# jimmyyhwu/spatial-intention-maps

Measured on AMD Instinct MI355X. Metric: Q-map transitions/sec, 96x96: `value` = full train() step (M2: policy fwd + bwd, double-DQN next-state forwards, clip, SGD); `value_fwd_bwd_only` = policy fwd+bwd alone (M1, the literal reading of "fwd+bwd"), higher is better.
Workload: dtype f32

## Files before the change

### include/simq.h

```cpp
#ifndef SIMQ_H
#define SIMQ_H

#include <stdint.h>

#ifdef __cplusplus
extern "C" {
#endif

#define SIMQ_VERSION 500
#define SIMQ_STATE_WIDTH 96

#define SIMQ_MODE_EVAL 0
#define SIMQ_MODE_TRAIN 1
#define SIMQ_MODE_TRAIN_NOGRAD 2

#define SIMQ_KIND_CONV_W 0
#define SIMQ_KIND_CONV_B 1
#define SIMQ_KIND_BN_W 2
#define SIMQ_KIND_BN_B 3

#define SIMQ_PREC_FP32 0
#define SIMQ_PREC_BF16X3 1
#define SIMQ_PREC_BF16 2

// ... 144 lines not shown
int simq_comm_broadcast(simq_comm* comm, void* d_buf, int64_t bytes, int root, void* producer_stream);
int simq_comm_wait(simq_comm* comm, void* consumer_stream);
int simq_comm_progress(simq_comm* comm, int64_t out[4]);
int simq_comm_time_waits(simq_comm* comm, int on);
int simq_comm_last_wait_ms(simq_comm* comm, float* ms);
int simq_comm_destroy(simq_comm* comm);

int simq_bce_with_logits(const float* d_logits, const float* d_target, int64_t n, float* d_dlogits, double* d_loss_sum, void* stream);
int simq_split_last_channel(const float* d_x, float* d_head, float* d_last, int64_t pixels, int channels, void* stream);
int simq_sigmoid_concat(const float* d_state, const float* d_logit, float* d_out, float* d_prob, int64_t pixels, int channels, void* stream);

int simq_nchw_to_nhwc(const float* d_in, float* d_out, int batch, int channels, int hw, void* stream);
int simq_nhwc_to_nchw(const float* d_in, float* d_out, int batch, int channels, int hw, void* stream);

typedef struct simq_launch_opts {
    int struct_bytes;
    int force_bm, force_bn;
    int tail_split;
    int plane_xcd;
    int wgrad_xcd_group;
    int wgrad_ksplit;
    int gemm_split;
} simq_launch_opts;
void simq_launch_opts_default(simq_launch_opts* opts);
int simq_conv2d_fwd(const float* d_x, const float* d_w_ohwi, const float* d_bias, float* d_y,
                    int batch, int hin, int win, int cin, int cout, int r, int s, int stride, int pad,
                    double* d_stats , void* stream, const simq_launch_opts* opts);
int simq_conv2d_fwd_winograd(const float* d_x, const float* d_w_ohwi, const float* d_bias, float* d_y,
                             int batch, int hin, int win, int cin, int cout,
                             double* d_stats , float* d_scratch, void* stream, const simq_launch_opts* opts);
int simq_conv2d_fwd_winograd4(const float* d_x, const float* d_w_ohwi, const float* d_bias, float* d_y,
                              int batch, int hin, int win, int cin, int cout,
                              double* d_stats , float* d_scratch, void* stream, const simq_launch_opts* opts);
int simq_bn_relu_apply(const void* d_y, const double* d_stats, const float* d_gamma, const float* d_beta, const void* d_res, int relu,
                       void* d_out, int64_t rows, int channels, int storage, float* d_saved, float* d_running, void* stream);
int simq_bn_relu_backward(const void* d_g, const void* d_mask, int mask_kind, const void* d_y, const float* d_saved, const float* d_gamma,
                          const double* d_red, void* d_dy, void* d_dz_out, float* d_dgamma, float* d_dbeta, int64_t rows, int channels,
                          int storage, void* stream);
int simq_conv2d_fwd_bnrelu_in(const float* d_y_pre, const float* d_in_scale, const float* d_in_shift, const float* d_w_ohwi,
                              const float* d_bias, float* d_y, int batch, int hin, int win, int cin, int cout, int r, int s, int stride,
                              int pad, int form, float* d_scratch, void* stream, const simq_launch_opts* opts);
int simq_conv2d_wgrad_bnrelu_in(const float* d_y_pre, const float* d_in_scale, const float* d_in_shift, const float* d_dy, float* d_dw,
                                int batch, int hin, int win, int cin, int cout, int r, int s, int stride, int pad, int form,
                                float* d_scratch, void* stream, const simq_launch_opts* opts);
int simq_conv2d_fwd_stem_f32(const float* d_x, const float* d_w_ohwi, float* d_y, int batch, int hin, int win, int cin, double* d_stats,
                             void* stream);
int simq_conv2d_fwd_stem_bf16(const float* d_x, const float* d_w_ohwi, uint16_t* d_y, int batch, int hin, int win, int cin,
                              double* d_stats, void* d_scratch, void* stream);
int simq_conv2d_wgrad_stem_bf16(const float* d_x, const uint16_t* d_dy, float* d_dw, int batch, int hin, int win, int cin,
                                float* d_scratch, void* stream);
int simq_conv2d_wgrad_winograd(const float* d_x, const float* d_dy, float* d_dw_ohwi,
                               int batch, int hin, int win, int cin, int cout, float* d_scratch, void* stream, const simq_launch_opts* opts);
int simq_gemm_f32_batched(const float* d_x, const float* d_w, float* d_y, int m, int n, int k, int batch, void* stream,
                          const simq_launch_opts* opts);
int simq_conv2d_dgrad(const float* d_dy, const float* d_w_ohwi, float* d_wt_scratch, float* d_dx,
                      int batch, int hin, int win, int cin, int cout, int r, int s, int pad, void* stream, const simq_launch_opts* opts);
int simq_conv2d_wgrad(const float* d_x, const float* d_dy, float* d_dw_ohwi ,
                      int batch, int hin, int win, int cin, int cout, int r, int s, int stride, int pad,
                      void* stream, const simq_launch_opts* opts);
int simq_conv2d_fwd_bf16(const float* d_x, const float* d_w_ohwi, const float* d_bias, float* d_y, int batch, int hin, int win,
                         int cin, int cout, int r, int s, int stride, int pad, int nplanes, void* d_scratch, double* d_stats,
                         void* stream, const simq_launch_opts* opts);
int simq_conv2d_wgrad_bf16(const float* d_x, const float* d_dy, float* d_dw_ohwi, int batch, int hin, int win, int cin, int cout,
                           int r, int s, int stride, int pad, int nplanes, void* d_scratch, void* stream, const simq_launch_opts* opts);
int64_t simq_conv2d_wgrad_bf16_slab_bytes(void);
int simq_conv2d_wgrad_bf16_slab(const float* d_x, const float* d_dy, float* d_dw_ohwi, int batch, int hin, int win, int cin, int cout,
// ... 185 lines not shown
```

### spatial-intention-maps_amd/csrc/common.h

```cpp
#pragma once
#include <hip/hip_runtime.h>
#include <stdint.h>

struct simq_comm;

namespace simq {

typedef float floatx16 __attribute__((ext_vector_type(16)));
typedef float floatx4 __attribute__((ext_vector_type(4)));

void set_error(const char* fmt, ...);

#ifdef SIMQ_ABLATIONS
int tune_env_int(const char* name, int dflt);
#define SIMQ_TUNE_INT(name, dflt) (simq::tune_env_int(name, dflt))
#else
#define SIMQ_TUNE_INT(name, dflt) (dflt)
#endif

#define SIMQ_CHECK_HIP(expr)                                                        \
    do {                                                                            \
        hipError_t _e = (expr);                                                     \
        if (_e != hipSuccess) {                                                     \
            simq::set_error("%s:%d: %s -> %s", __FILE__, __LINE__, #expr, hipGetErrorString(_e)); \
// ... 57 lines not shown
    int C = 0;
    double* defer = nullptr;
};
struct InBn {
    const float* scale = nullptr; const float* shift = nullptr;
    BnRef bn;
    int live = 0;
    bool on() const { return live != 0 || scale != nullptr; }
};

void prof_launch_begin(int kind, double flops, double bytes, hipStream_t stream);
void prof_launch_end(hipStream_t stream);
void note_launch(const char* family);

int launch_conv_igemm(const float* x, const float* w, float* y, const ConvGeom& g, const ConvEpilogue& e,
                      hipStream_t stream, const InBn& in = InBn());
int try_gemm_batched_pp(const float* x, const float* w, float* y, int M, int N, int K, int batch, hipStream_t stream);
int launch_gemm_batched(const float* x, const float* w, float* y, int M, int N, int K, int batch, hipStream_t stream, const LaunchTune& tune = LaunchTune());
bool gemm_split3_eligible(int M, int N, int K, int batch);
int launch_gemm_batched_split3(const float* x, const float* w, float* y, int M, int N, int K, int batch, hipStream_t stream, const LaunchTune& tune);
bool winograd_eligible(const ConvGeom& g);
bool winograd_pays(int cin, int cout, long min_cc);
int64_t winograd_scratch_floats(const ConvGeom& g);
int launch_wino_weight(const float* w_ohwi, float* U, int cout, int cin, hipStream_t stream);
struct WinoWeightDesc { int64_t src_off, u_off; int cout, cin, from_wt, pad_; };
constexpr int kWinoWeightTableCap = 72;
struct WinoWeightTable { WinoWeightDesc d[kWinoWeightTableCap]; int n; };
int launch_wino_weight_all(const float* params, const float* wt, float* ubase, const WinoWeightTable& t, hipStream_t stream);
int launch_conv_winograd(const float* x, const float* U, float* y, const ConvGeom& g, const ConvEpilogue& e, float* scratch,
                         hipStream_t stream, const InBn& in = InBn());
bool winograd_f4_forward(const ConvGeom& g, int min_tiles);
int launch_conv_winograd4(const float* x, const float* U4, float* y, const ConvGeom& g, const ConvEpilogue& e, float* scratch,
                          hipStream_t stream, const InBn& in = InBn());
constexpr int64_t kWgradDetSlabFloats = 16 << 20;
constexpr int kWgradMaxSplits = 96;
inline int64_t stem_det_slab_floats(int cin) {
    const int64_t want = (int64_t)kWgradMaxSplits * 64 * 49 * cin;
    return want < kWgradDetSlabFloats ? want : kWgradDetSlabFloats;
}
int launch_conv_wgrad(const float* x, const float* dy, float* dw, const ConvGeom& g, hipStream_t stream, const InBn& in = InBn(), float* det_slab = nullptr,
                      int64_t det_slab_floats = kWgradDetSlabFloats);
int launch_wgrad_slab_sum(const float* slab, float* dw, int64_t n, int splits, hipStream_t stream);
int launch_wgrad_batched(const float* x, const float* dy, float* dw, int M, int N, int K, int batch, hipStream_t stream, const LaunchTune& tune = LaunchTune());
bool winograd_wgrad_eligible(const ConvGeom& g);
bool winograd_wgrad_pays(const ConvGeom& g, bool allow_f4);
int launch_conv_wgrad_winograd(const float* x, const float* dy, float* dw, const ConvGeom& g, float* scratch, hipStream_t stream, bool allow_f4 = true,
                               const InBn& in = InBn());
int tune_forced_tile(const LaunchTune& t, int* bm, int* bn);
int launch_conv_igemm_bf16(const uint16_t* const x[2], const uint16_t* const w[2], int nplanes, float* y, const ConvGeom& g,
                           const ConvEpilogue& e, hipStream_t stream);
int launch_conv_wgrad_bf16(const uint16_t* const x[2], const uint16_t* const dy[2], int nplanes, float* dw, const ConvGeom& g,
                           hipStream_t stream, float* slab = nullptr, float* det_slab = nullptr);
int try_conv_wgrad_bf16_pp(const uint16_t* x, const uint16_t* dy, float* dw, const ConvGeom& g, unsigned x_bytes, unsigned dy_bytes,
                           hipStream_t stream);
int try_conv_wgrad_bf16_img(const uint16_t* x, const uint16_t* dy, float* dw, const ConvGeom& g, unsigned x_bytes, unsigned dy_bytes,
                           hipStream_t stream, float* slab = nullptr);
int64_t conv_wgrad_bf16_slab_bytes();
struct WeightPrepDesc { int64_t w_off, wt_off, wp_off; int cout, taps, cin, pad_; };
struct WeightPrepTable { WeightPrepDesc d[24]; int n; };
int launch_weight_prep_all(const float* params, const WeightPrepTable& t, float* wt_f32, uint16_t* wpl, uint16_t* wtpl, int np,
                           int64_t wp_total, hipStream_t stream);
int launch_split_planes(const float* src, uint16_t* hi, uint16_t* lo, int64_t n, hipStream_t stream);
int launch_weight_planes(const float* w, uint16_t* w_hi, uint16_t* w_lo, uint16_t* wt_hi, uint16_t* wt_lo, int cout, int taps,
                         int cin, hipStream_t stream);
int launch_weight_transpose(const float* w, float* wt, int cout, int taps, int cin, hipStream_t stream);

// ... 80 lines not shown
```

### spatial-intention-maps_amd/csrc/conv_winograd.hip

```cpp
#include "common.h"
#include "bn_coeff.h"
#include "igemm_epilogue.h"

namespace simq {

namespace {

__global__ void __launch_bounds__(256) wino_weight_kernel(const float* __restrict__ w, float* __restrict__ U, int cout, int cin) {
    const int total = cout * cin;
    for (int i = blockIdx.x * 256 + threadIdx.x; i < total; i += gridDim.x * 256) {
        const int co = i / cin, ci = i - co * cin;
        const float* g = w + (size_t)co * 9 * cin + ci;
        float t[4][3];
#pragma unroll
        for (int c = 0; c < 3; ++c) {
            const float g0 = g[(0 * 3 + c) * cin], g1 = g[(1 * 3 + c) * cin], g2 = g[(2 * 3 + c) * cin];
            t[0][c] = g0;
            t[1][c] = 0.5f * (g0 + g1 + g2);
            t[2][c] = 0.5f * (g0 - g1 + g2);
            t[3][c] = g2;
        }
#pragma unroll
        for (int r = 0; r < 4; ++r) {
            const float u0 = t[r][0], u1 = 0.5f * (t[r][0] + t[r][1] + t[r][2]), u2 = 0.5f * (t[r][0] - t[r][1] + t[r][2]), u3 = t[r][2];
// ... 324 lines not shown
                    }
                    s0 += dz;
                    s1 += dz * ((y1 - mu1) * is1);
                    if (bnr2) {
                        const floatx4 y2 = *reinterpret_cast<const floatx4*>(p.bnr_y2 + o);
                        s2 += dz;
                        s3 += dz * ((y2 - mu2) * is2);
                    }
                }
            }
        }
    }
    if (!p.stats && !bnr) return;
#pragma unroll
    for (int c = 0; c < 4; ++c) {
        red[0][threadIdx.x][c] = s0[c]; red[1][threadIdx.x][c] = s1[c];
        red[2][threadIdx.x][c] = s2[c]; red[3][threadIdx.x][c] = s3[c];
    }
    __syncthreads();
    for (int lc = threadIdx.x; lc < 4 * lanes; lc += 256) {
        double a0 = 0.0, a1 = 0.0, a2 = 0.0, a3 = 0.0;
        for (int k = 0; k < tpb; ++k) {
            const int src = k * lanes + (lc >> 2);
            a0 += (double)red[0][src][lc & 3]; a1 += (double)red[1][src][lc & 3];
            a2 += (double)red[2][src][lc & 3]; a3 += (double)red[3][src][lc & 3];
        }
        const int ch = blockIdx.y * lanes * 4 + lc;
        double* dst = p.stats ? p.stats : p.bnr_red1;
        unsafeAtomicAdd(dst + ch, a0);
        unsafeAtomicAdd(dst + C + ch, a1);
        if (bnr2) {
            unsafeAtomicAdd(p.bnr_red2 + ch, a2);
            unsafeAtomicAdd(p.bnr_red2 + C + ch, a3);
        }
    }
}

__global__ void __launch_bounds__(256) wino_dy_kernel(const float* __restrict__ dy, float* __restrict__ dM, int B, int H, int W, int C, int T) {
    const int lanes = C >> 2, tpb = 256 / lanes;
    const int cl = threadIdx.x % lanes, tl = threadIdx.x / lanes;
    const int th = H >> 1, tw = W >> 1;
    const size_t gstride = (size_t)T * C;
    for (int t = blockIdx.x * tpb + tl; t < T; t += gridDim.x * tpb) {
        const int b = t / (th * tw), r = t - b * (th * tw);
        const int ty = r / tw, tx = r - ty * tw;
        const float* src = dy + ((size_t)(b * H + 2 * ty) * W + 2 * tx) * C + cl * 4;
        const floatx4 y00 = *reinterpret_cast<const floatx4*>(src), y01 = *reinterpret_cast<const floatx4*>(src + C);
        const floatx4 y10 = *reinterpret_cast<const floatx4*>(src + (size_t)W * C), y11 = *reinterpret_cast<const floatx4*>(src + (size_t)W * C + C);
        floatx4 a[4][2];
        a[0][0] = y00; a[0][1] = y01;
        a[1][0] = y00 + y10; a[1][1] = y01 + y11;
        a[2][0] = y00 - y10; a[2][1] = y01 - y11;
        a[3][0] = -y10; a[3][1] = -y11;
        float* dst = dM + (size_t)t * C + cl * 4;
#pragma unroll
        for (int i = 0; i < 4; ++i) {
            *reinterpret_cast<floatx4*>(dst + (i * 4 + 0) * gstride) = a[i][0];
            *reinterpret_cast<floatx4*>(dst + (i * 4 + 1) * gstride) = a[i][0] + a[i][1];
            *reinterpret_cast<floatx4*>(dst + (i * 4 + 2) * gstride) = a[i][0] - a[i][1];
            *reinterpret_cast<floatx4*>(dst + (i * 4 + 3) * gstride) = -a[i][1];
        }
    }
}

template <bool DY, bool XBN = false>
__global__ void __launch_bounds__(256) wino_tr_kernel(const float* __restrict__ src, float* __restrict__ out, int B, int H, int W, int C, int T,
// ... 260 lines not shown
    if (bin > 4096) bin = 4096;
    if (in.on()) hipLaunchKernelGGL(wino_input_kernel<true>, dim3(bin), dim3(256), 0, stream, x, V, g.B, g.Hin, g.Win, g.Cin, T, in);
    else hipLaunchKernelGGL(wino_input_kernel<false>, dim3(bin), dim3(256), 0, stream, x, V, g.B, g.Hin, g.Win, g.Cin, T, in);
    SIMQ_CHECK_LAUNCH();
    if (int rc = launch_gemm_batched(V, U, Mt, T, g.Cout, g.Cin, 16, stream, g.tune)) return rc;
    int bout = (T + tpb_out - 1) / tpb_out;
    bout = balanced_grid(bout, (e.stats || e.bnr_red1) ? 512 : 4096);
    const EpiArgs ea = make_epi(y, e);
    note_launch("winograd_f2");
    hipLaunchKernelGGL(wino_output_kernel, dim3(bout), dim3(256), 0, stream, Mt, ea, g.B, g.Hin, g.Win, g.Cout, T);
    SIMQ_CHECK_LAUNCH();
    return 0;
}

bool winograd_f4_forward(const ConvGeom& g, int min_tiles) {
    return winograd_eligible(g) && g.Hin % 4 == 0 && g.Win % 4 == 0 && g.B * (g.Hin / 4) * (g.Win / 4) >= min_tiles;
}


int launch_conv_winograd4(const float* x, const float* U4, float* y, const ConvGeom& g, const ConvEpilogue& e, float* scratch,
                          hipStream_t stream, const InBn& in) {
    SIMQ_REQUIRE(winograd_eligible(g) && g.Hin % 4 == 0 && g.Win % 4 == 0, "conv_winograd4: geometry not supported");
    SIMQ_REQUIRE(!e.y_bf16, "conv_winograd4: fp32 outputs only");
    const int T4 = g.B * (g.Hin / 4) * (g.Win / 4);
    float* V = scratch;
    float* Mt = scratch + (size_t)36 * T4 * g.Cin;
    const int tpb_in = 256 / (g.Cin / 4);
    int bin = (T4 + tpb_in - 1) / tpb_in;
    if (bin > 4096) bin = 4096;
    if (in.on()) hipLaunchKernelGGL(wino4f_input_kernel<true>, dim3(bin), dim3(256), 0, stream, x, V, g.B, g.Hin, g.Win, g.Cin, T4, in);
    else hipLaunchKernelGGL(wino4f_input_kernel<false>, dim3(bin), dim3(256), 0, stream, x, V, g.B, g.Hin, g.Win, g.Cin, T4, in);
    SIMQ_CHECK_LAUNCH();
    if (int rc = launch_gemm_batched(V, U4, Mt, T4, g.Cout, g.Cin, 36, stream, g.tune)) return rc;
    static const int slice_quads = SIMQ_TUNE_INT("SIMQ_W4F_OUT_SLICE_QUADS", 16);
    int lanes_out = g.Cout / 4;
    if ((e.stats || e.bnr_red1) && slice_quads > 0 && lanes_out > slice_quads && lanes_out % slice_quads == 0) lanes_out = slice_quads;
    const int tpb_o = 256 / lanes_out, slices = (g.Cout / 4) / lanes_out;
    int bout = (T4 + tpb_o - 1) / tpb_o;
    bout = balanced_grid(bout, ((e.stats || e.bnr_red1) ? 1024 : 4096) / slices);
    const EpiArgs ea = make_epi(y, e);
    note_launch("winograd_f4");
    hipLaunchKernelGGL(wino4f_output_kernel, dim3(bout, slices), dim3(256), 0, stream, Mt, ea, g.B, g.Hin, g.Win, g.Cout, T4, lanes_out);
    SIMQ_CHECK_LAUNCH();
    return 0;
}

bool winograd_wgrad_eligible(const ConvGeom& g) { return winograd_eligible(g) && g.Cin % 128 == 0 && g.Cout % 128 == 0; }

bool winograd_wgrad_f4(const ConvGeom& g) {
    return g.Hin % 4 == 0 && g.Win % 4 == 0 && (g.B * (g.Hin / 4) * (g.Win / 4)) % 16 == 0;
}

bool winograd_wgrad_pays(const ConvGeom& g, bool allow_f4) {
    return (long)g.Cin * g.Cout >= ((allow_f4 && winograd_wgrad_f4(g)) ? 128L * 256 : 256L * 256);
}

int launch_conv_wgrad_winograd(const float* x, const float* dy, float* dw, const ConvGeom& g, float* scratch, hipStream_t stream, bool allow_f4,
                               const InBn& in) {
    SIMQ_REQUIRE(winograd_wgrad_eligible(g), "conv_wgrad_winograd: geometry not supported");
    const int T = g.B * (g.Hin / 2) * (g.Win / 2);
    float* Vt = scratch;
    float* dMt = scratch + (size_t)16 * T * g.Cin;
    float* dU = dMt + (size_t)16 * T * g.Cout;
    static const int direct_form = SIMQ_TUNE_INT("SIMQ_WINOGRAD_WGRAD_SPLITK", 0);
    const int T4 = g.B * (g.Hin / 4) * (g.Win / 4);
    if (!direct_form && allow_f4 && winograd_wgrad_f4(g)) {
        int S = 1;
        {
            const int ksplit = (g.tune.wgrad_ksplit == 1 || g.tune.wgrad_ksplit == 2 || g.tune.wgrad_ksplit == 4) ? g.tune.wgrad_ksplit : 0;
            const long blocks = 36L * (g.Cout / 64) * (g.Cin / 64);
            const long room = (long)winograd_scratch_floats(g) - 36L * T4 * (g.Cin + g.Cout);
            for (int cand = 4; cand >= 2; cand >>= 1) {
                if (ksplit > 0 && cand != ksplit) continue;
                const bool fits = T4 % (cand * 32) == 0 && 36L * (cand - 1) * g.Cout * g.Cin <= room;
                const int kc = T4 / cand;
// ... 51 lines not shown
```

### spatial-intention-maps_amd/csrc/ops_abi.hip

```cpp
#include "plan.h"

using namespace simq;

namespace {
int tune_of(const simq_launch_opts* o, LaunchTune* t) {
    *t = LaunchTune();
    if (!o) return 0;
    SIMQ_REQUIRE(o->struct_bytes == (int)sizeof(simq_launch_opts), "simq_launch_opts.struct_bytes = %d, this library's struct has %d (fill it with "
                 "simq_launch_opts_default first)", o->struct_bytes, (int)sizeof(simq_launch_opts));
    t->force_bm = o->force_bm > 0 ? o->force_bm : 0; t->force_bn = o->force_bm > 0 ? o->force_bn : 0;
    t->tail_split = o->tail_split; t->plane_xcd = o->plane_xcd; t->wgrad_xcd_group = o->wgrad_xcd_group; t->wgrad_ksplit = o->wgrad_ksplit;
    t->gemm_split = o->gemm_split;
    return 0;
}
}

extern "C" {

int simq_q_argmax(const float* d_q, int rows, int n, int64_t* d_index, float* d_max, void* stream) {
    SIMQ_REQUIRE(rows >= 0 && n >= 1, "q_argmax: bad shape");
    return launch_q_argmax(d_q, rows, n, d_index, d_max, static_cast<hipStream_t>(stream));
}

int simq_q_gather(const float* d_q, int rows, int n, const int64_t* d_index, float* d_out, void* stream) {
// ... 170 lines not shown
int simq_conv2d_fwd_stem_bf16(const float* d_x, const float* d_w, uint16_t* d_y, int batch, int hin, int win, int cin, double* d_stats,
                              void* d_scratch, void* stream) {
    SIMQ_REQUIRE(d_x && d_w && d_y && d_scratch && batch >= 1, "conv2d_fwd_stem_bf16: bad argument");
    SIMQ_REQUIRE(stem_conv_bf16_eligible(hin, win, cin, 64, 7, 2, 3), "conv2d_fwd_stem_bf16: geometry not supported (7 * cin <= 63, win %% 32 == 0)");
    hipStream_t st = static_cast<hipStream_t>(stream);
    RC(launch_stem_weight_prep(d_w, static_cast<uint16_t*>(d_scratch), cin, st));
    return launch_stem_conv_bf16(d_x, static_cast<const uint16_t*>(d_scratch), d_y, d_stats, batch, hin, win, cin, st);
}

int simq_conv2d_wgrad_stem_bf16(const float* d_x, const uint16_t* d_dy, float* d_dw, int batch, int hin, int win, int cin, float* d_scratch,
                                void* stream) {
    SIMQ_REQUIRE(d_x && d_dy && d_dw && d_scratch && batch >= 1, "conv2d_wgrad_stem_bf16: bad argument");
    SIMQ_REQUIRE(stem_conv_bf16_eligible(hin, win, cin, 64, 7, 2, 3), "conv2d_wgrad_stem_bf16: geometry not supported (7 * cin <= 63, win %% 32 == 0)");
    return launch_stem_wgrad_bf16(d_x, d_dy, d_dw, d_scratch, batch, hin, win, cin, static_cast<hipStream_t>(stream));
}

int simq_conv2d_fwd_winograd4(const float* d_x, const float* d_w, const float* d_bias, float* d_y, int batch, int hin, int win,
                              int cin, int cout, double* d_stats, float* d_scratch, void* stream, const simq_launch_opts* opts) {
    SIMQ_REQUIRE(d_x && d_w && d_y && d_scratch && batch >= 1, "conv2d_fwd_winograd4: bad argument");
    ConvGeom g;
    RC(tune_of(opts, &g.tune));
    g.B = batch; g.Hin = hin; g.Win = win; g.Cin = cin; g.Cout = cout; g.R = 3; g.S = 3; g.stride = 1; g.pad = 1; g.Hout = hin; g.Wout = win;
    SIMQ_REQUIRE(winograd_eligible(g) && hin % 4 == 0 && win % 4 == 0, "conv2d_fwd_winograd4: geometry not supported (map %% 4, cin %% 16, cout %% 64)");
    ConvEpilogue e;
    e.bias = d_bias; e.stats = d_stats;
    hipStream_t st = static_cast<hipStream_t>(stream);
    WinoWeightTable t;
    t.n = 1;
    t.d[0] = WinoWeightDesc{0, 0, cout, cin, 0, 1};
    RC(launch_wino_weight_all(d_w, nullptr, d_scratch, t, st));
    return launch_conv_winograd4(d_x, d_scratch, d_y, g, e, d_scratch + (size_t)36 * cout * cin, st);
}

int simq_conv2d_wgrad_winograd(const float* d_x, const float* d_dy, float* d_dw, int batch, int hin, int win, int cin, int cout,
                               float* d_scratch, void* stream, const simq_launch_opts* opts) {
    SIMQ_REQUIRE(d_x && d_dy && d_dw && d_scratch && batch >= 1, "conv2d_wgrad_winograd: bad argument");
    ConvGeom g;
    RC(tune_of(opts, &g.tune));
    g.B = batch; g.Hin = hin; g.Win = win; g.Cin = cin; g.Cout = cout; g.R = 3; g.S = 3; g.stride = 1; g.pad = 1; g.Hout = hin; g.Wout = win;
    SIMQ_REQUIRE(winograd_wgrad_eligible(g), "conv2d_wgrad_winograd: geometry not supported (even map, cin %% 128, cout %% 128)");
    return launch_conv_wgrad_winograd(d_x, d_dy, d_dw, g, d_scratch, static_cast<hipStream_t>(stream));
}

int simq_gemm_f32_batched(const float* d_x, const float* d_w, float* d_y, int m, int n, int k, int batch, void* stream, const simq_launch_opts* opts) {
    SIMQ_REQUIRE(d_x && d_w && d_y, "gemm_f32_batched: NULL argument");
    LaunchTune t;
    RC(tune_of(opts, &t));
    return launch_gemm_batched(d_x, d_w, d_y, m, n, k, batch, static_cast<hipStream_t>(stream), t);
}

int simq_conv2d_dgrad(const float* d_dy, const float* d_w, float* d_wt_scratch, float* d_dx, int batch, int hin, int win,
                      int cin, int cout, int r, int s, int pad, void* stream, const simq_launch_opts* opts) {
    hipStream_t st = static_cast<hipStream_t>(stream);
    SIMQ_REQUIRE(r == s, "conv2d_dgrad: square filters only");
    RC(launch_weight_transpose(d_w, d_wt_scratch, cout, r * s, cin, st));
    ConvGeom g;
    RC(tune_of(opts, &g.tune));
    g.B = batch; g.Hin = hin; g.Win = win; g.Cin = cout; g.Cout = cin; g.Hout = hin; g.Wout = win;
    g.R = r; g.S = s; g.stride = 1; g.pad = r - 1 - pad;
    ConvEpilogue e;
    return launch_conv_igemm(d_dy, d_wt_scratch, d_dx, g, e, st);
}

int simq_conv2d_wgrad(const float* d_x, const float* d_dy, float* d_dw, int batch, int hin, int win, int cin, int cout,
                      int r, int s, int stride, int pad, void* stream, const simq_launch_opts* opts) {
    hipStream_t st = static_cast<hipStream_t>(stream);
// ... 66 lines not shown
```

### spatial-intention-maps_amd/simq/_lib.py

```python
import ctypes
import os
from ctypes import POINTER, c_char_p, c_double, c_float, c_int, c_int64, c_void_p

import torch

_HERE = os.path.dirname(os.path.abspath(__file__))
LIB_PATH = os.environ.get('SIMQ_LIBRARY') or os.path.join(_HERE, 'libsimq.so')

MODE_EVAL, MODE_TRAIN, MODE_TRAIN_NOGRAD = 0, 1, 2
KIND_CONV_W, KIND_CONV_B, KIND_BN_W, KIND_BN_B = 0, 1, 2, 3
PRECISIONS = {'fp32': 0, 'bf16x3': 1, 'bf16': 2}
COMM_ID_BYTES, COMM_F32, COMM_F64 = 128, 0, 1


class SimqError(RuntimeError):
    pass


if not os.path.exists(LIB_PATH):
    raise SimqError('libsimq.so not found at %s -- build it with `python -c "import __graft_entry__ as g; g.build()"` '
                    '(or `make -C spatial-intention-maps_amd/csrc`); there is no CPU fallback' % LIB_PATH)

_c = ctypes.CDLL(LIB_PATH)

REDUCE_FN = ctypes.CFUNCTYPE(c_int, c_void_p, c_void_p, c_int64, c_void_p)


class SyncArgs(ctypes.Structure):
    _fields_ = [('reduce', REDUCE_FN), ('user', c_void_p), ('global_batch', c_int), ('world_size', c_int)]


class PlanOptions(ctypes.Structure):
    _fields_ = [(n, c_int) for n in (
        'struct_bytes', 'winograd', 'winograd_min_cc', 'winograd_f4_forward', 'winograd_f4_min_tiles', 'winograd_f4_grad',
        'winograd_f4_fwd_grad_min_cc', 'winograd_wgrad', 'winograd_wgrad_f4', 'stem_bf16', 'bf16_act_grads', 'keep_fp32_activations', 'fold_eval_bn_bf16',
        'fuse_bn_backward_sums', 'fuse_stem_backward_sums', 'fuse_bn1_apply', 'deterministic', 'bn1_mask_from_preact',
        'wgrad_ksplit', 'fwd_overlap', 'wgrad_overlap', 'plane_xcd', 'wgrad_xcd_group', 'tail_split', 'early_target_after_block', 'gemm_split')]


class LaunchOpts(ctypes.Structure):
    _fields_ = [(n, c_int) for n in ('struct_bytes', 'force_bm', 'force_bn', 'tail_split', 'plane_xcd', 'wgrad_xcd_group', 'wgrad_ksplit', 'gemm_split')]


class TrainArgs(ctypes.Structure):
    _fields_ = [('plan', c_void_p),
                ('batch', c_int), ('num_nonfinal', c_int), ('global_batch', c_int), ('use_double_dqn', c_int), ('first_step', c_int),
                ('sync_bn', c_int),
                ('gamma', c_float), ('lr', c_float), ('momentum', c_float), ('weight_decay', c_float), ('max_norm', c_float),
                ('reserved2_', c_float)] + [(n, c_void_p) for n in (
                    'params', 'wcache', 'bnbuf', 'grads', 'momentum_buf', 'ws_train', 'ws_tmp',
                    't_params', 't_wcache', 't_bnbuf', 't_ws',
                    'state', 'next_state', 'action', 'reward', 'nonfinal_pos',
                    'q', 'q_next', 'q_tgt', 'dq', 'nsv', 'vals', 'best', 'q_sa', 'y', 'td', 'out4',
                    'opt_scratch', 'total_norm', 'stream', 'side_stream')] + [('global_nonfinal', c_int), ('struct_bytes', c_int), ('comm', c_void_p), ('loss_host', c_void_p), ('target_stream', c_void_p), ('third_stream', c_void_p)]


_SIGS = {
    'simq_version': (c_int, []),
    'simq_build_flags': (c_int, []),
    'simq_last_error': (c_char_p, []),
    'simq_plan_create': (c_int, [c_int, c_int, POINTER(c_void_p)]),
    'simq_plan_create_ex': (c_int, [c_int, c_int, c_int, POINTER(c_void_p)]),
    'simq_plan_options_default': (None, [c_void_p]),
    'simq_launch_opts_default': (None, [c_void_p]),
    'simq_plan_create_opts': (c_int, [c_int, c_int, c_int, c_void_p, POINTER(c_void_p)]),
    'simq_plan_get_options': (c_int, [c_void_p, c_void_p]),
    'simq_plan_precision': (c_int, [c_void_p]),
    'simq_plan_destroy': (None, [c_void_p]),
    'simq_param_count': (c_int64, [c_void_p]),
    'simq_param_num_tensors': (c_int, [c_void_p]),
    'simq_param_tensor_info': (c_int, [c_void_p, c_int, c_char_p, c_int, POINTER(c_int64), POINTER(c_int64 * 4), POINTER(c_int)]),
    'simq_bnbuf_count': (c_int64, [c_void_p]),
    'simq_bn_num_layers': (c_int, [c_void_p]),
    'simq_bn_layer_info': (c_int, [c_void_p, c_int, c_char_p, c_int, POINTER(c_int64), POINTER(c_int)]),
# ... 17 lines not shown
    'simq_q_argmax': (c_int, [c_void_p, c_int, c_int, c_void_p, c_void_p, c_void_p]),
    'simq_q_gather': (c_int, [c_void_p, c_int, c_int, c_void_p, c_void_p, c_void_p]),
    'simq_scatter_next_values': (c_int, [c_void_p, c_void_p, c_int, c_void_p, c_int, c_void_p]),
    'simq_td_huber': (c_int, [c_void_p, c_int, c_int, c_void_p, c_void_p, c_void_p, c_float, c_float,
                              c_void_p, c_void_p, c_void_p, c_void_p, c_void_p, c_void_p]),
    'simq_clip_sgd_step': (c_int, [c_void_p, c_void_p, c_void_p, c_int64, c_float, c_float, c_float, c_float, c_int,
                                   c_void_p, c_void_p, c_void_p]),
    'simq_bce_with_logits': (c_int, [c_void_p, c_void_p, c_int64, c_void_p, c_void_p, c_void_p]),
    'simq_split_last_channel': (c_int, [c_void_p, c_void_p, c_void_p, c_int64, c_int, c_void_p]),
    'simq_sigmoid_concat': (c_int, [c_void_p, c_void_p, c_void_p, c_void_p, c_int64, c_int, c_void_p]),
    'simq_replay_gather': (c_int, [c_void_p, c_int64, c_void_p, c_int, c_void_p, c_void_p]),
    'simq_replay_scatter': (c_int, [c_void_p, c_int64, c_void_p, c_int, c_void_p, c_int64, c_void_p, c_int64, c_void_p]),
    'simq_nchw_to_nhwc': (c_int, [c_void_p, c_void_p, c_int, c_int, c_int, c_void_p]),
    'simq_nhwc_to_nchw': (c_int, [c_void_p, c_void_p, c_int, c_int, c_int, c_void_p]),
    'simq_conv2d_fwd': (c_int, [c_void_p, c_void_p, c_void_p, c_void_p] + [c_int] * 9 + [c_void_p, c_void_p] + [c_void_p]),
    'simq_gemm_f32_batched': (c_int, [c_void_p, c_void_p, c_void_p, c_int, c_int, c_int, c_int, c_void_p, c_void_p]),
    'simq_conv2d_dgrad': (c_int, [c_void_p, c_void_p, c_void_p, c_void_p] + [c_int] * 8 + [c_void_p] + [c_void_p]),
    'simq_conv2d_wgrad': (c_int, [c_void_p, c_void_p, c_void_p] + [c_int] * 9 + [c_void_p] + [c_void_p]),
    'simq_conv2d_fwd_bf16': (c_int, [c_void_p, c_void_p, c_void_p, c_void_p] + [c_int] * 10 + [c_void_p, c_void_p, c_void_p] + [c_void_p]),
    'simq_conv2d_wgrad_bf16': (c_int, [c_void_p, c_void_p, c_void_p] + [c_int] * 10 + [c_void_p, c_void_p] + [c_void_p]),
    'simq_conv2d_wgrad_bf16_slab_bytes': (c_int64, []),
    'simq_conv2d_wgrad_bf16_slab': (c_int, [c_void_p, c_void_p, c_void_p] + [c_int] * 10 + [c_void_p, c_void_p, c_void_p] + [c_void_p]),
    'simq_wgrad_slab_sum': (c_int, [c_void_p, c_void_p, c_int64, c_int, c_void_p]),
    'simq_upsample2x_fwd': (c_int, [c_void_p, c_void_p, c_int, c_int, c_int, c_int, c_void_p]),
    'simq_upsample2x_bwd': (c_int, [c_void_p, c_void_p, c_int, c_int, c_int, c_int, c_void_p]),
    'simq_profile_start': (c_int, []),
    'simq_profile_stop': (c_int, [c_void_p, c_int]),
    'simq_launch_counts_reset': (c_int, []),
    'simq_launch_count': (c_int64, [c_char_p]),
    'simq_launch_counts': (c_int, [c_char_p, c_int]),
    'simq_conv2d_wgrad_winograd': (c_int, [c_void_p, c_void_p, c_void_p] + [c_int] * 5 + [c_void_p, c_void_p] + [c_void_p]),
    'simq_conv2d_fwd_winograd': (c_int, [c_void_p, c_void_p, c_void_p, c_void_p] + [c_int] * 5 + [c_void_p, c_void_p, c_void_p] + [c_void_p]),
    'simq_conv2d_fwd_winograd4': (c_int, [c_void_p, c_void_p, c_void_p, c_void_p] + [c_int] * 5 + [c_void_p, c_void_p, c_void_p] + [c_void_p]),
    'simq_bn_relu_apply': (c_int, [c_void_p] * 5 + [c_int, c_void_p, c_int64, c_int, c_int, c_void_p, c_void_p, c_void_p]),
    'simq_bn_relu_backward': (c_int, [c_void_p, c_void_p, c_int] + [c_void_p] * 8 + [c_int64, c_int, c_int, c_void_p]),
    'simq_conv2d_fwd_bnrelu_in': (c_int, [c_void_p] * 6 + [c_int] * 10 + [c_void_p, c_void_p] + [c_void_p]),
    'simq_conv2d_wgrad_bnrelu_in': (c_int, [c_void_p] * 5 + [c_int] * 10 + [c_void_p, c_void_p] + [c_void_p]),
    'simq_conv2d_fwd_stem_f32': (c_int, [c_void_p, c_void_p, c_void_p] + [c_int] * 4 + [c_void_p, c_void_p]),
    'simq_conv2d_fwd_stem_bf16': (c_int, [c_void_p, c_void_p, c_void_p] + [c_int] * 4 + [c_void_p, c_void_p, c_void_p]),
    'simq_conv2d_wgrad_stem_bf16': (c_int, [c_void_p, c_void_p, c_void_p] + [c_int] * 4 + [c_void_p, c_void_p]),
    'simq_forward_sync': (c_int, [c_void_p, c_int, c_int, c_void_p, c_void_p, c_void_p, c_void_p, c_void_p, c_void_p, c_void_p, c_void_p]),
    'simq_backward_sync': (c_int, [c_void_p, c_int, c_void_p, c_void_p, c_void_p, c_void_p, c_void_p, c_void_p, c_float, c_void_p, c_void_p,
                                   c_int, c_void_p, c_void_p]),
    'simq_comm_reduce_f64': (c_int, [c_void_p, c_void_p, c_int64, c_void_p]),
    'simq_forward_sync_null': (c_int, [c_void_p, c_int, c_void_p, c_void_p, c_void_p, c_void_p]),
    'simq_comm_unique_id': (c_int, [c_void_p]),
    'simq_comm_init': (c_int, [c_void_p, c_int, c_int, POINTER(c_void_p)]),
    'simq_comm_adopt_stream': (c_int, [c_void_p, c_void_p]),
    'simq_comm_world_size': (c_int, [c_void_p]),
    'simq_comm_rank': (c_int, [c_void_p]),
    'simq_comm_allreduce': (c_int, [c_void_p, c_void_p, c_int64, c_int, c_void_p]),
    'simq_comm_broadcast': (c_int, [c_void_p, c_void_p, c_int64, c_int, c_void_p]),
    'simq_comm_wait': (c_int, [c_void_p, c_void_p]),
    'simq_comm_progress': (c_int, [c_void_p, c_void_p]),
    'simq_comm_time_waits': (c_int, [c_void_p, c_int]),
    'simq_comm_last_wait_ms': (c_int, [c_void_p, POINTER(c_float)]),
    'simq_comm_destroy': (c_int, [c_void_p]),
    'simq_grid_distance_images': (c_int, [c_void_p, c_int64, c_void_p, c_int, c_void_p, c_void_p, c_int64, c_float, c_int, c_float,
                                          c_void_p, c_void_p]),
    'simq_grid_distance_images_snapped': (c_int, [c_void_p, c_int64, c_void_p, c_int64, c_void_p, c_int, c_void_p, c_void_p, c_int64, c_float,
                                                  c_int, c_float, c_void_p, c_int, c_void_p, c_void_p]),
    'simq_grid_paths': (c_int, [c_void_p, c_int64, c_void_p, c_int64, c_void_p, c_int, c_void_p, c_void_p, c_int64, c_void_p, c_void_p, c_void_p,
                                c_int64, c_void_p, c_int64, c_void_p, c_void_p]),
    'simq_grid_distance_queries': (c_int, [c_void_p, c_int64, c_void_p, c_int64, c_void_p, c_int, c_void_p, c_int64, c_void_p, c_void_p, c_int64,
                                           c_int, c_void_p, c_int64, c_void_p, c_void_p]),
    'simq_local_state_desc_bytes': (c_int64, [c_int, c_int, c_int, c_int]),
# ... 3 lines not shown
    'simq_local_state_images_slots': (c_int, [c_void_p, c_int, c_void_p, c_int, c_void_p, c_int, c_void_p, c_int, c_void_p, c_int, c_void_p, c_void_p,
                                              c_int64, c_void_p, c_int64, c_void_p]),
    'simq_intention_desc_bytes': (c_int64, [c_int, c_int]),
    'simq_intention_maps': (c_int, [c_void_p, c_int, c_void_p, c_int, c_int, c_int, c_int, c_void_p, c_int64, c_void_p, c_int64, c_void_p]),
    'simq_occupancy_maps': (c_int, [c_void_p, c_int64, c_void_p, c_int, c_void_p, c_void_p, c_void_p, c_int64, c_void_p, c_int64, c_void_p,
                                    c_void_p]),
    'simq_observation_update': (c_int, [c_void_p, c_int64, c_void_p, c_int, c_void_p, c_void_p, c_int64, c_void_p, c_int64, c_void_p, c_void_p]),
    'simq_state_output_visualizations': (c_int, [c_void_p, c_int, c_void_p, c_void_p, c_double, c_int, c_void_p, c_int64, c_void_p]),
}

EXPORTS = tuple(_SIGS)
OPTS_FUNCS = frozenset(('simq_gemm_f32_batched', 'simq_conv2d_fwd', 'simq_conv2d_dgrad', 'simq_conv2d_wgrad', 'simq_conv2d_fwd_bf16', 'simq_conv2d_wgrad_bf16',
                        'simq_conv2d_wgrad_bf16_slab', 'simq_conv2d_wgrad_winograd', 'simq_conv2d_fwd_winograd', 'simq_conv2d_fwd_winograd4',
                        'simq_conv2d_fwd_bnrelu_in', 'simq_conv2d_wgrad_bnrelu_in'))


def launch_counts():
    buf = ctypes.create_string_buffer(4096)
    check(_c.simq_launch_counts(buf, 4096), 'simq_launch_counts')
    return {kv.split('=')[0]: int(kv.split('=')[1]) for kv in buf.value.decode().split(';') if kv}


def launch_opts(tile=None, **fields):
    o = LaunchOpts()
    _c.simq_launch_opts_default(ctypes.byref(o))
    if tile is not None and tile[0] > 0:
        o.force_bm, o.force_bn = int(tile[0]), int(tile[1])
    for k, v in fields.items():
        if k == 'struct_bytes' or not hasattr(o, k):
            raise SimqError('unknown launch option %r (fields of simq_launch_opts: %s)' % (k, ', '.join(n for n, _ in LaunchOpts._fields_[1:])))
        setattr(o, k, int(v))
    return o

for _name, (_res, _args) in _SIGS.items():
    _fn = getattr(_c, _name)
    _fn.restype = _res
    _fn.argtypes = _args


def last_error():
    return (_c.simq_last_error() or b'').decode()


def check(rc, what):
    if rc != 0:
        raise SimqError('%s failed (%d): %s' % (what, rc, last_error()))


def ptr(t):
    return None if t is None else c_void_p(t.data_ptr())


def stream_ptr(device=None):
    return c_void_p(torch.cuda.current_stream(device).cuda_stream)


class Lib:
    c = _c
    version = _c.simq_version()
    build_flags = _c.simq_build_flags()
    path = LIB_PATH


    @staticmethod
    def call(name, *args, opts=None):
        if name in OPTS_FUNCS:
# ... 67 lines not shown
```

Baseline: 4738.

## Add two-phase Winograd F4 output kernel with row-staged epilogue loads

Adds a new Winograd F(4,3) output-transform kernel, templated on the epilogue form. Each thread loads all 36 transform values for a tile at once, does the inverse transform, then stages the addend, mask and BN-input loads in row groups sized to fit the register budget, overlapping them with the epilogue math of earlier rows. The conv path now defaults to this kernel (form 1) and falls back to the old per-pixel kernel for very large tensors or when stats and BN-reduction are both requested. A standalone ABI and Python entry point expose it for testing. The cost is higher register pressure and more template instantiations.

Result: faster. 4848 (median of 6 runs) (+2.3%).

```diff
diff --git a/include/simq.h b/include/simq.h
--- a/include/simq.h
+++ b/include/simq.h
@@ -200,6 +200,16 @@
 int simq_conv2d_fwd_winograd4(const float* d_x, const float* d_w_ohwi, const float* d_bias, float* d_y,
                               int batch, int hin, int win, int cin, int cout,
                               double* d_stats , float* d_scratch, void* stream, const simq_launch_opts* opts);
+typedef struct simq_wino4f_epilogue {
+    int struct_bytes;
+    int relu;
+    const float* bias; double* stats; const float* scale; const float* shift; const float* addend;
+    const float* bnr_mask; const uint16_t* bnr_mask16; const float* bnr_mscale; const float* bnr_mshift;
+    const float* bnr_y1; const float* bnr_mean1; const float* bnr_invstd1; double* bnr_red1;
+    const float* bnr_y2; const float* bnr_mean2; const float* bnr_invstd2; double* bnr_red2;
+} simq_wino4f_epilogue;
+int simq_wino4f_output(const float* d_mt, float* d_y, int batch, int h, int w, int channels, const simq_wino4f_epilogue* epilogue,
+                       int form, void* stream);
 int simq_bn_relu_apply(const void* d_y, const double* d_stats, const float* d_gamma, const float* d_beta, const void* d_res, int relu,
                        void* d_out, int64_t rows, int channels, int storage, float* d_saved, float* d_running, void* stream);
 int simq_bn_relu_backward(const void* d_g, const void* d_mask, int mask_kind, const void* d_y, const float* d_saved, const float* d_gamma,
diff --git a/spatial-intention-maps_amd/csrc/common.h b/spatial-intention-maps_amd/csrc/common.h
--- a/spatial-intention-maps_amd/csrc/common.h
+++ b/spatial-intention-maps_amd/csrc/common.h
@@ -113,6 +113,7 @@
 bool winograd_f4_forward(const ConvGeom& g, int min_tiles);
 int launch_conv_winograd4(const float* x, const float* U4, float* y, const ConvGeom& g, const ConvEpilogue& e, float* scratch,
                           hipStream_t stream, const InBn& in = InBn());
+int launch_wino4f_output(const float* Mt, float* y, const ConvEpilogue& e, int B, int H, int W, int C, int form, hipStream_t stream);
 constexpr int64_t kWgradDetSlabFloats = 16 << 20;
 constexpr int kWgradMaxSplits = 96;
 inline int64_t stem_det_slab_floats(int cin) {
diff --git a/spatial-intention-maps_amd/csrc/conv_winograd.hip b/spatial-intention-maps_amd/csrc/conv_winograd.hip
--- a/spatial-intention-maps_amd/csrc/conv_winograd.hip
+++ b/spatial-intention-maps_amd/csrc/conv_winograd.hip
@@ -380,6 +380,167 @@
         if (bnr2) {
             unsafeAtomicAdd(p.bnr_red2 + ch, a2);
             unsafeAtomicAdd(p.bnr_red2 + C + ch, a3);
+        }
+    }
+}
+
+template <bool ADD, int BNR, bool Y2>
+constexpr int w4f_out_rows() {
+    const int per_pixel = (ADD ? 4 : 0) + (BNR ? 4 : 0) + (BNR == 1 ? 4 : BNR == 2 ? 2 : 0) + (Y2 ? 4 : 0);
+    return per_pixel * 16 <= 96 ? 4 : per_pixel * 8 <= 96 ? 2 : 1;
+}
+
+template <bool ADD, int BNR, bool Y2, bool STATS, int ABL>
+__global__ void __launch_bounds__(256, 2) wino4f_output2_kernel(const float* __restrict__ Mt, const EpiArgs p, int B, int H, int W, int C, int T, int lanes) {
+    static_assert(BNR >= 0 && BNR <= 3 && (BNR != 0 || !Y2) && !(STATS && BNR != 0), "wino4f_output2_kernel: form");
+    constexpr bool LDS = STATS || BNR != 0;
+    constexpr int ROWS = w4f_out_rows<ADD, BNR, Y2>();
+    constexpr bool LOADS = !(ABL & 4);
+    const int tpb = 256 / lanes;
+    const int cl = threadIdx.x % lanes, tl = threadIdx.x / lanes;
+    const int th = H >> 2, tw = W >> 2;
+    const size_t gstride = (size_t)T * C;
+    const int n = (blockIdx.y * lanes + cl) * 4;
+    constexpr bool bnr = BNR != 0, bnr2 = Y2;
+    const bool relu = p.relu != 0;
+    floatx4 bias = {0.f, 0.f, 0.f, 0.f}, sc = {1.f, 1.f, 1.f, 1.f}, sh = bias, mu1 = bias, is1 = bias, mu2 = bias, is2 = bias, msc = bias, msh = bias;
+#pragma unroll
+    for (int c = 0; c < 4; ++c) {
+        if (p.bias) bias[c] = p.bias[n + c];
+        if (p.scale) { sc[c] = p.scale[n + c]; sh[c] = p.shift[n + c]; }
+        if (bnr) { mu1[c] = p.bnr_mean1[n + c]; is1[c] = p.bnr_invstd1[n + c]; }
+        if (BNR == 3 && p.bnr_mscale) { msc[c] = p.bnr_mscale[n + c]; msh[c] = p.bnr_mshift[n + c]; }
+        if (bnr2) { mu2[c] = p.bnr_mean2[n + c]; is2[c] = p.bnr_invstd2[n + c]; }
+    }
+    floatx4 s0 = {0.f, 0.f, 0.f, 0.f}, s1 = s0, s2 = s0, s3 = s0;
+    for (int t = blockIdx.x * tpb + tl; t < T; t += gridDim.x * tpb) {
+        const int b = t / (th * tw), r = t - b * (th * tw);
+        const int ty = r / tw, tx = r - ty * tw;
+        const float* src = Mt + (size_t)t * C + n;
+        floatx4 v[4][4];
+        {
+            floatx4 mt[6][6];
+#pragma unroll
+            for (int g = 0; g < 36; ++g) mt[g % 6][g / 6] = *reinterpret_cast<const floatx4*>(src + g * gstride);
+            __builtin_amdgcn_sched_barrier(0);
+            floatx4 a[4][6];
+#pragma unroll
+            for (int j = 0; j < 6; ++j) {
+                floatx4 m[6], y[4];
+#pragma unroll
+                for (int i = 0; i < 6; ++i) m[i] = mt[j][i];
+                w4f_at(m, y);
+#pragma unroll
+                for (int i = 0; i < 4; ++i) a[i][j] = y[i];
+            }
+#pragma unroll
+            for (int i = 0; i < 4; ++i) {
+                floatx4 y[4];
+                w4f_at(a[i], y);
+#pragma unroll
+                for (int j = 0; j < 4; ++j) v[i][j] = y[j] + bias;
+            }
+        }
+        const unsigned o00 = (unsigned)((((size_t)(b * H + 4 * ty) * W + 4 * tx) * C + n) * sizeof(float));
+        auto f4 = [&](const float* base, int i, int j) {
+            return reinterpret_cast<const floatx4*>(reinterpret_cast<const char*>(base + ((size_t)i * W + j) * C) + o00);
+        };
+        floatx4 ad[4][4], y1[4][4], mk[4][4], y2[4][4];
+        ushort4 mk16[4][4];
+        auto load_rows = [&](int i0) {
+            __builtin_amdgcn_sched_barrier(0);
+#pragma unroll
+            for (int i = i0; i < i0 + ROWS; ++i)
+#pragma unroll
+                for (int j = 0; j < 4; ++j) {
+                    if constexpr (LOADS) {
+                        if constexpr (ADD) ad[i][j] = *f4(p.addend, i, j);
+                        if constexpr (bnr) y1[i][j] = *f4(p.bnr_y1, i, j);
+                        if constexpr (BNR == 1) mk[i][j] = *f4(p.bnr_mask, i, j);
+                        if constexpr (BNR == 2)
+                            mk16[i][j] = *reinterpret_cast<const ushort4*>(reinterpret_cast<const char*>(p.bnr_mask16 + ((size_t)i * W + j) * C) + (o00 >> 1));
+                        if constexpr (bnr2) y2[i][j] = *f4(p.bnr_y2, i, j);
+                    } else {
+                        ad[i][j] = y1[i][j] = mk[i][j] = y2[i][j] = v[i][j];
+                        mk16[i][j] = make_ushort4(1, 1, 1, 1);
+                    }
+                }
+            __builtin_amdgcn_sched_barrier(0);
+        };
+        load_rows(0);
+#pragma unroll
+        for (int i0 = 0; i0 < 4; i0 += ROWS) {
+#pragma unroll
+            for (int i = i0; i < i0 + ROWS; ++i)
+#pragma unroll
+                for (int j = 0; j < 4; ++j) {
+                    floatx4 v_ = v[i][j];
+                    if constexpr (STATS && !(ABL & 2)) { s0 += v_; s1 += v_ * v_; }
+                    v_ = v_ * sc + sh;
+                    if constexpr (ADD) v_ += ad[i][j];
+#pragma unroll
+                    for (int c = 0; c < 4; ++c) v_[c] = relu ? fmaxf(v_[c], 0.f) : v_[c];
+                    v[i][j] = v_;
+                    if constexpr (bnr) {
+                        floatx4 dz;
+                        if constexpr (BNR == 1) {
+#pragma unroll
+                            for (int c = 0; c < 4; ++c) dz[c] = mk[i][j][c] > 0.f ? v_[c] : 0.f;
+                        } else if constexpr (BNR == 2) {
+                            const ushort4 m16 = mk16[i][j];
+                            dz[0] = (short)m16.x > 0 ? v_[0] : 0.f; dz[1] = (short)m16.y > 0 ? v_[1] : 0.f;
+                            dz[2] = (short)m16.z > 0 ? v_[2] : 0.f; dz[3] = (short)m16.w > 0 ? v_[3] : 0.f;
+                        } else {
+#pragma unroll
+                            for (int c = 0; c < 4; ++c) dz[c] = __builtin_fmaf(y1[i][j][c], msc[c], msh[c]) > 0.f ? v_[c] : 0.f;
+                        }
+                        if constexpr (!(ABL & 2)) {
+                            s0 += dz;
+                            s1 += dz * ((y1[i][j] - mu1) * is1);
+                            if constexpr (bnr2) {
+                                s2 += dz;
+                                s3 += dz * ((y2[i][j] - mu2) * is2);
+                            }
+                        } else {
+                            asm volatile("" :: "v"(dz[0]), "v"(dz[1]), "v"(dz[2]), "v"(dz[3]));
+                        }
+                    }
+                }
+            if (i0 + ROWS < 4) load_rows(i0 + ROWS);
+            else __builtin_amdgcn_sched_barrier(0);
+#pragma unroll
+            for (int i = i0; i < i0 + ROWS; ++i)
+#pragma unroll
+                for (int j = 0; j < 4; ++j) *const_cast<floatx4*>(f4(p.y, i, j)) = v[i][j];
+        }
+    }
+    if constexpr (LDS && !(ABL & 2)) {
+        __shared__ float red[4][256][4];
+#pragma unroll
+        for (int c = 0; c < 4; ++c) {
+            red[0][threadIdx.x][c] = s0[c]; red[1][threadIdx.x][c] = s1[c];
+            red[2][threadIdx.x][c] = s2[c]; red[3][threadIdx.x][c] = s3[c];
+        }
+        __syncthreads();
+        for (int lc = threadIdx.x; lc < 4 * lanes; lc += 256) {
+            double a0 = 0.0, a1 = 0.0, a2 = 0.0, a3 = 0.0;
+            for (int k = 0; k < tpb; ++k) {
+                const int src = k * lanes + (lc >> 2);
+                a0 += (double)red[0][src][lc & 3]; a1 += (double)red[1][src][lc & 3];
+                a2 += (double)red[2][src][lc & 3]; a3 += (double)red[3][src][lc & 3];
+            }
+            if constexpr (ABL & 1) {
+                asm volatile("" :: "v"(a0), "v"(a1), "v"(a2), "v"(a3));
+            } else {
+                const int ch = blockIdx.y * lanes * 4 + lc;
+                double* dst = STATS ? p.stats : p.bnr_red1;
+                unsafeAtomicAdd(dst + ch, a0);
+                unsafeAtomicAdd(dst + C + ch, a1);
+                if (bnr2) {
+                    unsafeAtomicAdd(p.bnr_red2 + ch, a2);
+                    unsafeAtomicAdd(p.bnr_red2 + C + ch, a3);
+                }
+            }
         }
     }
 }
@@ -706,15 +867,54 @@
     else hipLaunchKernelGGL(wino4f_input_kernel<false>, dim3(bin), dim3(256), 0, stream, x, V, g.B, g.Hin, g.Win, g.Cin, T4, in);
     SIMQ_CHECK_LAUNCH();
     if (int rc = launch_gemm_batched(V, U4, Mt, T4, g.Cout, g.Cin, 36, stream, g.tune)) return rc;
+    return launch_wino4f_output(Mt, y, e, g.B, g.Hin, g.Win, g.Cout, 1, stream);
+}
+
+template <int ABL>
+static void launch_wino4f_output2(dim3 grid, hipStream_t stream, const float* Mt, const EpiArgs& ea, int B, int H, int W, int C, int T4, int lanes) {
+    const bool add = ea.addend != nullptr, y2 = ea.bnr_red1 && ea.bnr_red2, stats = ea.stats != nullptr;
+    const int bnr = !ea.bnr_red1 ? 0 : ea.bnr_mask ? 1 : ea.bnr_mask16 ? 2 : 3;
+#define SIMQ_W4F_OUT2(ADD, BNR, Y2, STATS)                                                                                                      \
+    if (add == ADD && bnr == BNR && y2 == Y2 && stats == STATS) {                                                                                 \
+        hipLaunchKernelGGL((wino4f_output2_kernel<ADD, BNR, Y2, STATS, ABL>), grid, dim3(256), 0, stream, Mt, ea, B, H, W, C, T4, lanes);       \
+        return;                                                                                                                                 \
+    }
+#define SIMQ_W4F_OUT2_ADD(ADD)                                                                                                                  \
+    SIMQ_W4F_OUT2(ADD, 0, false, false); SIMQ_W4F_OUT2(ADD, 0, false, true);                                                                    \
+    SIMQ_W4F_OUT2(ADD, 1, false, false); SIMQ_W4F_OUT2(ADD, 1, true, false); SIMQ_W4F_OUT2(ADD, 2, false, false); SIMQ_W4F_OUT2(ADD, 2, true, false); \
+    SIMQ_W4F_OUT2(ADD, 3, false, false); SIMQ_W4F_OUT2(ADD, 3, true, false)
+    SIMQ_W4F_OUT2_ADD(false);
+    SIMQ_W4F_OUT2_ADD(true);
+#undef SIMQ_W4F_OUT2_ADD
+#undef SIMQ_W4F_OUT2
+}
+
+int launch_wino4f_output(const float* Mt, float* y, const ConvEpilogue& e, int B, int H, int W, int C, int form, hipStream_t stream) {
+    SIMQ_REQUIRE(Mt && y && B >= 1 && H >= 4 && W >= 4 && H % 4 == 0 && W % 4 == 0 && C >= 4 && C % 4 == 0 && C / 4 <= 256 && 256 % (C / 4) == 0,
+                 "wino4f_output: geometry not supported (map %% 4, C / 4 divides 256)");
+    SIMQ_REQUIRE(!e.y_bf16 && !(e.addend && e.addend_bf16) && !(e.bnr_red1 && e.bnr_y_bf16), "wino4f_output: fp32 tensors only");
+    SIMQ_REQUIRE(!e.bnr_red1 || (e.bnr_y1 && e.bnr_mean1 && e.bnr_invstd1), "wino4f_output: bnr_red1 without bnr_y1 / bnr_mean1 / bnr_invstd1");
+    SIMQ_REQUIRE(!(e.bnr_red1 && e.bnr_red2) || (e.bnr_y2 && e.bnr_mean2 && e.bnr_invstd2), "wino4f_output: bnr_red2 without bnr_y2 / bnr_mean2 / bnr_invstd2");
+    SIMQ_REQUIRE(!e.scale == !e.shift && !e.bnr_mscale == !e.bnr_mshift, "wino4f_output: scale / shift come in pairs");
+    const int T4 = B * (H / 4) * (W / 4);
     static const int slice_quads = SIMQ_TUNE_INT("SIMQ_W4F_OUT_SLICE_QUADS", 16);
-    int lanes_out = g.Cout / 4;
+    int lanes_out = C / 4;
     if ((e.stats || e.bnr_red1) && slice_quads > 0 && lanes_out > slice_quads && lanes_out % slice_quads == 0) lanes_out = slice_quads;
-    const int tpb_o = 256 / lanes_out, slices = (g.Cout / 4) / lanes_out;
+    const int tpb_o = 256 / lanes_out, slices = (C / 4) / lanes_out;
     int bout = (T4 + tpb_o - 1) / tpb_o;
     bout = balanced_grid(bout, ((e.stats || e.bnr_red1) ? 1024 : 4096) / slices);
     const EpiArgs ea = make_epi(y, e);
     note_launch("winograd_f4");
-    hipLaunchKernelGGL(wino4f_output_kernel, dim3(bout, slices), dim3(256), 0, stream, Mt, ea, g.B, g.Hin, g.Win, g.Cout, T4, lanes_out);
+    const dim3 grid(bout, slices);
+    if (form == 1 && ((double)B * H * W * C * sizeof(float) >= 4294967296.0 || (e.stats && e.bnr_red1))) form = 0;
+    if (form == 0) hipLaunchKernelGGL(wino4f_output_kernel, grid, dim3(256), 0, stream, Mt, ea, B, H, W, C, T4, lanes_out);
+    else if (form == 1) launch_wino4f_output2<0>(grid, stream, Mt, ea, B, H, W, C, T4, lanes_out);
+#ifdef SIMQ_ABLATIONS
+    else if (form == 1 + 16 * 1) launch_wino4f_output2<1>(grid, stream, Mt, ea, B, H, W, C, T4, lanes_out);
+    else if (form == 1 + 16 * 2) launch_wino4f_output2<2>(grid, stream, Mt, ea, B, H, W, C, T4, lanes_out);
+    else if (form == 1 + 16 * 4) launch_wino4f_output2<4>(grid, stream, Mt, ea, B, H, W, C, T4, lanes_out);
+#endif
+    else SIMQ_REQUIRE(false, "wino4f_output: form %d (0: one pixel at a time, 1: two-phase)", form);
     SIMQ_CHECK_LAUNCH();
     return 0;
 }
diff --git a/spatial-intention-maps_amd/csrc/ops_abi.hip b/spatial-intention-maps_amd/csrc/ops_abi.hip
--- a/spatial-intention-maps_amd/csrc/ops_abi.hip
+++ b/spatial-intention-maps_amd/csrc/ops_abi.hip
@@ -226,6 +226,19 @@
     return launch_conv_winograd4(d_x, d_scratch, d_y, g, e, d_scratch + (size_t)36 * cout * cin, st);
 }
 
+int simq_wino4f_output(const float* d_mt, float* d_y, int batch, int h, int w, int channels, const simq_wino4f_epilogue* ep, int form, void* stream) {
+    SIMQ_REQUIRE(d_mt && d_y && ep, "wino4f_output: NULL argument");
+    SIMQ_REQUIRE(ep->struct_bytes == (int)sizeof(simq_wino4f_epilogue), "simq_wino4f_epilogue.struct_bytes = %d, this library's struct has %d",
+                 ep->struct_bytes, (int)sizeof(simq_wino4f_epilogue));
+    SIMQ_REQUIRE(batch >= 1 && h >= 4 && w >= 4 && channels >= 4 && (double)batch * h * w * channels < 2147483648.0, "wino4f_output: bad shape");
+    ConvEpilogue e;
+    e.bias = ep->bias; e.stats = ep->stats; e.scale = ep->scale; e.shift = ep->shift; e.addend = ep->addend; e.relu = ep->relu;
+    e.bnr_mask = ep->bnr_mask; e.bnr_mask16 = ep->bnr_mask16; e.bnr_mscale = ep->bnr_mscale; e.bnr_mshift = ep->bnr_mshift;
+    e.bnr_y1 = ep->bnr_y1; e.bnr_mean1 = ep->bnr_mean1; e.bnr_invstd1 = ep->bnr_invstd1; e.bnr_red1 = ep->bnr_red1;
+    e.bnr_y2 = ep->bnr_y2; e.bnr_mean2 = ep->bnr_mean2; e.bnr_invstd2 = ep->bnr_invstd2; e.bnr_red2 = ep->bnr_red2;
+    return launch_wino4f_output(d_mt, d_y, e, batch, h, w, channels, form, static_cast<hipStream_t>(stream));
+}
+
 int simq_conv2d_wgrad_winograd(const float* d_x, const float* d_dy, float* d_dw, int batch, int hin, int win, int cin, int cout,
                                float* d_scratch, void* stream, const simq_launch_opts* opts) {
     SIMQ_REQUIRE(d_x && d_dy && d_dw && d_scratch && batch >= 1, "conv2d_wgrad_winograd: bad argument");
diff --git a/spatial-intention-maps_amd/simq/_lib.py b/spatial-intention-maps_amd/simq/_lib.py
--- a/spatial-intention-maps_amd/simq/_lib.py
+++ b/spatial-intention-maps_amd/simq/_lib.py
@@ -40,6 +40,12 @@
 
 class LaunchOpts(ctypes.Structure):
     _fields_ = [(n, c_int) for n in ('struct_bytes', 'force_bm', 'force_bn', 'tail_split', 'plane_xcd', 'wgrad_xcd_group', 'wgrad_ksplit', 'gemm_split')]
+
+
+class Wino4fEpilogue(ctypes.Structure):
+    _fields_ = [('struct_bytes', c_int), ('relu', c_int)] + [(n, c_void_p) for n in (
+        'bias', 'stats', 'scale', 'shift', 'addend', 'bnr_mask', 'bnr_mask16', 'bnr_mscale', 'bnr_mshift',
+        'bnr_y1', 'bnr_mean1', 'bnr_invstd1', 'bnr_red1', 'bnr_y2', 'bnr_mean2', 'bnr_invstd2', 'bnr_red2')]
 
 
 class TrainArgs(ctypes.Structure):
@@ -123,6 +129,7 @@
     'simq_conv2d_wgrad_winograd': (c_int, [c_void_p, c_void_p, c_void_p] + [c_int] * 5 + [c_void_p, c_void_p] + [c_void_p]),
     'simq_conv2d_fwd_winograd': (c_int, [c_void_p, c_void_p, c_void_p, c_void_p] + [c_int] * 5 + [c_void_p, c_void_p, c_void_p] + [c_void_p]),
     'simq_conv2d_fwd_winograd4': (c_int, [c_void_p, c_void_p, c_void_p, c_void_p] + [c_int] * 5 + [c_void_p, c_void_p, c_void_p] + [c_void_p]),
+    'simq_wino4f_output': (c_int, [c_void_p, c_void_p, c_int, c_int, c_int, c_int, c_void_p, c_int, c_void_p]),
     'simq_bn_relu_apply': (c_int, [c_void_p] * 5 + [c_int, c_void_p, c_int64, c_int, c_int, c_void_p, c_void_p, c_void_p]),
     'simq_bn_relu_backward': (c_int, [c_void_p, c_void_p, c_int] + [c_void_p] * 8 + [c_int64, c_int, c_int, c_void_p]),
     'simq_conv2d_fwd_bnrelu_in': (c_int, [c_void_p] * 6 + [c_int] * 10 + [c_void_p, c_void_p] + [c_void_p]),
@@ -192,6 +199,18 @@
         setattr(o, k, int(v))
     return o
 
+def wino4f_output(mt, y, form=1, relu=False, **tensors):
+    e = Wino4fEpilogue()
+    e.struct_bytes, e.relu = ctypes.sizeof(Wino4fEpilogue), int(bool(relu))
+    for k, t in tensors.items():
+        if k in ('struct_bytes', 'relu') or not hasattr(e, k):
+            raise SimqError('unknown field %r of simq_wino4f_epilogue' % k)
+        setattr(e, k, None if t is None else t.data_ptr())
+    B, H, W, C = y.shape
+    check(_c.simq_wino4f_output(ptr(mt), ptr(y), B, H, W, C, ctypes.byref(e), int(form), stream_ptr(y.device)), 'simq_wino4f_output')
+    return y
+
+
 for _name, (_res, _args) in _SIGS.items():
     _fn = getattr(_c, _name)
     _fn.restype = _res
```
